# tphakala/birdnet-go

Hardware: AMD Instinct MI355X
Metric: 3s-48kHz clips/sec (whole node) + max-abs prob diff vs TFLite, BirdNET v2.4 (higher is better)
Workload: dtype f32; 1 GPU; BASELINE configs[1]: BirdNET v2.4 fp32, batch 256 x 3 s @ 48 kHz per GPU, mel front-end + CNN + head on device, raw logits out; batch_per_gpu=256, n_samples=144000, n_classes=6522, pipeline_depth=2, input_sets=4

## Files before the change

birdnet-go_amd/csrc/expdw.hip:

```cpp
#include "kernels.h"
#include "pw_common.h"

#include <algorithm>
#include <type_traits>
#include <cmath>
#include <cstdio>
#include <cstdlib>
#include <cstring>
#include <vector>

namespace bnhip {

struct ExpDwParams {
    const float* x; const float* we; const float* be; const float* wd; const float* bd;
    float* y; float* partial;
    int B, H, W, Cin, Cmid, Ho, Wo, pt, pl, act_e, act_d, tiles_h, tiles_w, cchunks, Kw, Cp;
    int Hin = 0, Win = 0, pts = 0, pls = 0;
    const uint16_t* wep = nullptr; int Kp = 0;
    int prec = 0;
    int xsh = 0, xsw = 1, ysh = 0, ysw = 1, tr = 0;
    int in_bf16 = 0, out_bf16 = 0;
    FDiv d_bpc{}, d_cch{}, d_tw{};
    int cpp = 0;
    FDiv d_part{};
// ... 48 lines not shown
            for (int j = 0; j < K; j++) w[j] = wds[(i * K + j) * 8 + c4];
#pragma unroll
            for (int a = 0; a < SH; a++) {
                const int fr = (ty * SH + a) * S + i;
                if (fr < vr0 || fr >= vr1 || oh0 + ty * SH + a >= p.Ho) continue;
                float4 xr[RW];
#pragma unroll
                for (int c = 0; c < RW; c++) xr[c] = *reinterpret_cast<const float4*>(e0 + ((fr - vr0) * TIW + c) * ED_ES);
#pragma unroll
                for (int j = 0; j < K; j++) {
#pragma unroll
                    for (int c = 0; c < SW; c++) {
                        const float4 xv = xr[c * S + j];
                        acc2[a][c].x = fmaf(xv.x, w[j].x, acc2[a][c].x); acc2[a][c].y = fmaf(xv.y, w[j].y, acc2[a][c].y);
                        acc2[a][c].z = fmaf(xv.z, w[j].z, acc2[a][c].z); acc2[a][c].w = fmaf(xv.w, w[j].w, acc2[a][c].w);
                    }
                }
            }
        }
    }
    pre_store();
    if (n < p.Cmid) {
        float* const yclip = p.y + (size_t)b * p.Ho * p.Wo * p.Cmid;
        const unsigned ylane = (unsigned)(((oh0 + ty * SH) * p.ysh + (ow0 + tx * SW) * p.ysw) * p.Cmid + n);
#pragma unroll
        for (int a = 0; a < SH; a++) {
            int oh = oh0 + ty * SH + a;
            if (oh >= p.Ho) continue;
            if (p.act_d == ACT_SWISH) {
#pragma unroll
                for (int c = 0; c < SW; c++) {
                    float4& v = acc2[a][c];
                    const f32x4 r = swish4((f32x4){v.x + bv.x, v.y + bv.y, v.z + bv.z, v.w + bv.w});
                    v = make_float4(r[0], r[1], r[2], r[3]);
                }
            } else {
                with_act(p.act_d, [&](auto f) {
#pragma unroll
                    for (int c = 0; c < SW; c++) {
                        float4& v = acc2[a][c];
                        v.x = f(v.x + bv.x); v.y = f(v.y + bv.y); v.z = f(v.z + bv.z); v.w = f(v.w + bv.w);
                    }
                });
            }
#pragma unroll
            for (int c = 0; c < SW; c++) {
                int ow = ow0 + tx * SW + c;
                if (ow >= p.Wo) continue;
                float4 v = acc2[a][c];
                const unsigned yo = ylane + (unsigned)((a * p.ysh + c * p.ysw) * p.Cmid);
                if (p.out_bf16) bf16x4_store(p.y, ((size_t)b * p.Ho * p.Wo * p.Cmid + yo) >> 2, v);
                else *reinterpret_cast<float4*>(yclip + yo) = v;
                sum.x += v.x; sum.y += v.y; sum.z += v.z; sum.w += v.w;
            }
        }
    }
    return sum;
}
__device__ __forceinline__ void ed_sums_lanes(float4 sum, float4* red, int wave, int lane, int c4) {
    static_assert(ed_perm_c4_rule(ED_PERM2) && ed_perm_c4_rule(ED_PERM4), "lane permutation: c4 bit 2 must be physical lane bit 3");
    auto xsum = [&](auto pat) {
        constexpr int P = decltype(pat)::value;
        sum.x += __builtin_bit_cast(float, __builtin_amdgcn_ds_swizzle(__builtin_bit_cast(int, sum.x), P));
        sum.y += __builtin_bit_cast(float, __builtin_amdgcn_ds_swizzle(__builtin_bit_cast(int, sum.y), P));
        sum.z += __builtin_bit_cast(float, __builtin_amdgcn_ds_swizzle(__builtin_bit_cast(int, sum.z), P));
        sum.w += __builtin_bit_cast(float, __builtin_amdgcn_ds_swizzle(__builtin_bit_cast(int, sum.w), P));
    };
    xsum(std::integral_constant<int, 0x101f>{});
    xsum(std::integral_constant<int, 0x401f>{});
    if ((lane & 0x14) == 0) red[(wave * 2 + (lane >> 5)) * 8 + c4] = sum;
}
template <int NW = 4>
__device__ __forceinline__ void ed_sums_out(const ExpDwParams& p, const float4* red, int tid, size_t tile_index, int n_base) {
    if (tid < 8 && n_base + 4 * tid < p.Cmid) {
        float4 t = red[tid];
#pragma unroll
        for (int w = 1; w < 2 * NW; w++) { float4 v = red[w * 8 + tid]; t.x += v.x; t.y += v.y; t.z += v.z; t.w += v.w; }
        unsigned l4 = 4u * (unsigned)tid;
        asm volatile("" : "+v"(l4));
        *reinterpret_cast<float4*>(p.partial + tile_index * p.Cmid + n_base + l4) = t;
    }
}

template <int K, int S, int TOH, int TOW, int TRH, bool H8 = false, bool BX = false, bool COPY = false>
__global__ __launch_bounds__(256, BX ? expdw_min_waves(K, S, TOW, TRH) : 1) void k_expand_dw(ExpDwParams p, unsigned nblk) {
    constexpr int TIH = (TOH - 1) * S + K, TIW = (TOW - 1) * S + K;
    static_assert(TRH <= TIH, "TRH is a cap on the footprint rows");
    constexpr int NPIX = TRH * TIW, NPIXP = (NPIX + 15) / 16 * 16;
    constexpr int JT = NPIXP / 16, JTW = (JT + 3) / 4;
    constexpr int SW = TOW / 8;
    __shared__ __attribute__((aligned(16))) float lds[NPIX * ED_ES + 256 + K * K * 32];
    float* E = lds;
    float4* red = reinterpret_cast<float4*>(lds + NPIX * ED_ES);
    float4* wds = reinterpret_cast<float4*>(lds + NPIX * ED_ES + 256);
    const int tid = threadIdx.x, lane = tid & 63, wave = __builtin_amdgcn_readfirstlane(tid >> 6);
    const int li = lane & 15, kq = lane >> 4;

    const unsigned L = xcd_remap(blockIdx.x, nblk);
    const int tiles = p.tiles_h * p.tiles_w;
    const int bpc = tiles * p.cchunks;
    const int b = (int)fdiv(L, p.d_bpc), rest = (int)L - b * bpc;
    const int tile = (int)fdiv((unsigned)rest, p.d_cch), cc = rest - tile * p.cchunks;
    const int trow = (int)fdiv((unsigned)tile, p.d_tw);
    const int oh0 = trow * TOH, ow0 = (tile - trow * p.tiles_w) * TOW;
    const int ih0 = oh0 * S - p.pt, iw0 = ow0 * S - p.pl;
    const int vr0 = max(ih0, 0) - ih0, vr1 = min(ih0 + TIH, p.H) - ih0;
    const int nvalid = (vr1 - vr0) * TIW;
    const int jtv = (nvalid + 15) >> 4;
    const int Cin = p.Cin, Kw = p.Kw;
    const int n_base = cc * 32;

    static_assert(SW * S == 2 || SW * S == 4, "lane permutation tables cover SW*S in {2, 4}");
    constexpr unsigned long long PERM = SW * S == 2 ? ED_PERM2 : ED_PERM4;
    const int pl = ed_perm(PERM, lane);
    const int c4 = pl & 7, tx = pl >> 3;
    float4 wdreg = make_float4(0.f, 0.f, 0.f, 0.f);
    if (tid < K * K * 8 && (!COPY || n_base + 4 * (tid & 7) < p.Cmid)) {
        const int tap = tid >> 3, tsrc = p.tr ? (tap % K) * K + tap / K : tap;
        wdreg = *reinterpret_cast<const float4*>(p.wd + (size_t)tsrc * p.Cp + n_base + 4 * (tid & 7));
    }
    const float4 zero4 = make_float4(0.f, 0.f, 0.f, 0.f);
    const float4 bq0 = COPY ? zero4 : *reinterpret_cast<const float4*>(p.be + n_base + 4 * kq);
    const float4 bq1 = COPY ? zero4 : *reinterpret_cast<const float4*>(p.be + n_base + 16 + 4 * kq);
    const float4 bv = (COPY && (!p.bd || n_base + 4 * c4 >= p.Cmid)) ? zero4 : *reinterpret_cast<const float4*>(p.bd + n_base + 4 * c4);

    if constexpr (COPY) {
        const float4* x4 = reinterpret_cast<const float4*>(p.x);
        const int C4 = p.Cmid >> 2, q4 = (n_base >> 2) + (tid & 7);
        const bool cin = q4 < C4;
        const size_t img = (size_t)b * p.H * p.W;
#pragma unroll 4
        for (int j = tid >> 3; j < nvalid; j += 32) {
            const int r = j / TIW, c = j - r * TIW;
            const int iw = iw0 + c, ih = ih0 + vr0 + r;
            float4 v = zero4;
            if (cin && iw >= 0 && iw < p.W) {
                const size_t quad = (img + (size_t)ih * p.xsh + (size_t)iw * p.xsw) * C4 + q4;
                v = p.in_bf16 ? bf16x4_load(p.x, quad) : x4[quad];
            }
            *reinterpret_cast<float4*>(&E[j * ED_ES + 4 * (tid & 7)]) = v;
        }
        if (tid < K * K * 8) wds[tid] = wdreg;
        __syncthreads();
    } else {

    int xoff[JTW];
    bool xin[JTW];
#pragma unroll
    for (int a = 0; a < JTW; a++) {
        int j = 16 * (wave + 4 * a) + li;
        int r = j / TIW, c = j - r * TIW;
        int iw = iw0 + c;
        xin[a] = j < nvalid && iw >= 0 && iw < p.W;
        int ihc = min(ih0 + vr0 + r, p.H - 1), iwc = min(max(iw, 0), p.W - 1);
        xoff[a] = (b * p.H * p.W + ihc * p.xsh + iwc * p.xsw) * Cin + (BX ? 8 : 4) * kq;
    }
    const float* wrow0 = p.we + (size_t)(n_base + li) * Kw + 4 * kq;
    const float* wrow1 = wrow0 + (size_t)16 * Kw;

    f32x4 acc[JTW][2];
#pragma unroll
    for (int a = 0; a < JTW; a++) { acc[a][0] = (f32x4){bq0.x, bq0.y, bq0.z, bq0.w}; acc[a][1] = (f32x4){bq1.x, bq1.y, bq1.z, bq1.w}; }

    auto fload = [&](int k0, f32x4& wf0, f32x4& wf1, f32x4 (&xf)[JTW]) {
        float4 t0 = *reinterpret_cast<const float4*>(wrow0 + k0), t1 = *reinterpret_cast<const float4*>(wrow1 + k0);
        wf0 = (f32x4){t0.x, t0.y, t0.z, t0.w}; wf1 = (f32x4){t1.x, t1.y, t1.z, t1.w};
        const int kx = (k0 + 4 * kq < Cin) ? k0 : -4 * kq;
#pragma unroll
        for (int a = 0; a < JTW; a++) {
            float4 t = *reinterpret_cast<const float4*>(p.x + (size_t)xoff[a] + kx);
            xf[a] = (f32x4){t.x, t.y, t.z, t.w};
        }
    };
    auto fmma = [&](const f32x4& wf0, const f32x4& wf1, const f32x4 (&xf)[JTW]) {
#pragma unroll
        for (int a = 0; a < JTW; a++) {
            if (wave + 4 * a < jtv) {
#pragma unroll
                for (int sidx = 0; sidx < 4; sidx++) {
                    acc[a][0] = __builtin_amdgcn_mfma_f32_16x16x4f32(wf0[sidx], xf[a][sidx], acc[a][0], 0, 0, 0);
                    acc[a][1] = __builtin_amdgcn_mfma_f32_16x16x4f32(wf1[sidx], xf[a][sidx], acc[a][1], 0, 0, 0);
                }
            }
        }
    };
    auto fload8 = [&](int k0, f32x2& wh0, f32x2& wh1, f32x2 (&xh)[JTW]) {
        const float2 t0 = *reinterpret_cast<const float2*>(wrow0 - 2 * kq + k0), t1 = *reinterpret_cast<const float2*>(wrow1 - 2 * kq + k0);
        wh0 = (f32x2){t0.x, t0.y}; wh1 = (f32x2){t1.x, t1.y};
        const int kx = (k0 + 2 * kq + 1 < Cin) ? k0 - 2 * kq : -4 * kq;
#pragma unroll
        for (int a = 0; a < JTW; a++) {
            const float2 t = *reinterpret_cast<const float2*>(p.x + (size_t)xoff[a] + kx);
            xh[a] = (f32x2){t.x, t.y};
        }
    };
    auto fmma8 = [&](const f32x2& wh0, const f32x2& wh1, const f32x2 (&xh)[JTW]) {
#pragma unroll
        for (int a = 0; a < JTW; a++) {
            if (wave + 4 * a < jtv) {
#pragma unroll
                for (int sidx = 0; sidx < 2; sidx++) {
                    acc[a][0] = __builtin_amdgcn_mfma_f32_16x16x4f32(wh0[sidx], xh[a][sidx], acc[a][0], 0, 0, 0);
                    acc[a][1] = __builtin_amdgcn_mfma_f32_16x16x4f32(wh1[sidx], xh[a][sidx], acc[a][1], 0, 0, 0);
                }
            }
        }
    };
    const int Kfull = Kw & ~15;
    if (BX) {
        const u32x4* wimg = reinterpret_cast<const u32x4*>(p.wep);
        const unsigned kp8 = (unsigned)p.Kp >> 3;
        const unsigned wr0 = (unsigned)(n_base + li) * 3u * kp8 + (unsigned)kq, wr1 = wr0 + 48u * kp8;
        for (int s32 = 0; s32 < (p.Kp >> 5); s32++) {
            const int kx = (32 * s32 + 8 * kq + 7 < Cin) ? 32 * s32 : -8 * kq;
            if (p.prec == 1) {
                const bf16x8 w0 = __builtin_bit_cast(bf16x8, wimg[wr0 + 4 * s32]), w1 = __builtin_bit_cast(bf16x8, wimg[wr1 + 4 * s32]);
#pragma unroll
                for (int a = 0; a < JTW; a++) {
                    if (wave + 4 * a < jtv) {
                        const float* xq = p.x + (size_t)xoff[a] + kx;
                        const float4 t0 = *reinterpret_cast<const float4*>(xq), t1 = *reinterpret_cast<const float4*>(xq + 4);
                        const bf16x8 xh = bx1_cvt8(t0, t1);
                        acc[a][0] = __builtin_amdgcn_mfma_f32_16x16x32_bf16(w0, xh, acc[a][0], 0, 0, 0);
                        acc[a][1] = __builtin_amdgcn_mfma_f32_16x16x32_bf16(w1, xh, acc[a][1], 0, 0, 0);
                    }
                }
                continue;
            }
            u32x4 wq[2][3];
#pragma unroll
            for (int pl3 = 0; pl3 < 3; pl3++) { wq[0][pl3] = wimg[wr0 + pl3 * kp8 + 4 * s32]; wq[1][pl3] = wimg[wr1 + pl3 * kp8 + 4 * s32]; }
#pragma unroll
            for (int a = 0; a < JTW; a++) {
                if (wave + 4 * a < jtv) {
                    const float* xq = p.x + (size_t)xoff[a] + kx;
                    const float4 t0 = *reinterpret_cast<const float4*>(xq), t1 = *reinterpret_cast<const float4*>(xq + 4);
                    bf16x8 xh, xm, xl;
                    bx3_split8(t0, t1, &xh, &xm, &xl);
#pragma unroll
                    for (int t = 0; t < 2; t++) {
                        acc[a][t] = bx3_mfma6(acc[a][t], __builtin_bit_cast(bf16x8, wq[t][0]), __builtin_bit_cast(bf16x8, wq[t][1]),
                                              __builtin_bit_cast(bf16x8, wq[t][2]), xh, xm, xl);
                    }
                }
            }
        }
    } else if (!H8) {
        for (int k0 = 0; k0 < Kw; k0 += 16) {
            f32x4 wf0, wf1, xf[JTW];
            fload(k0, wf0, wf1, xf);
            fmma(wf0, wf1, xf);
        }
    } else {
        for (int k0 = 0; k0 < Kfull; k0 += 16) {
            f32x4 wf0, wf1, xf[JTW];
            fload(k0, wf0, wf1, xf);
            fmma(wf0, wf1, xf);
        }
        f32x2 hA0, hA1, hx[JTW];
        fload8(Kfull, hA0, hA1, hx);
        fmma8(hA0, hA1, hx);
    }

    const bool border = iw0 < 0 || iw0 + TIW > p.W;
#pragma unroll
    for (int a = 0; a < JTW; a++) {
        if (wave + 4 * a < jtv) {
            if (p.act_e == ACT_SWISH) {
                acc[a][0] = swish4(acc[a][0]);
                acc[a][1] = swish4(acc[a][1]);
            } else {
                with_act(p.act_e, [&](auto f) {
                    f32x4& v0 = acc[a][0];
                    f32x4& v1 = acc[a][1];
                    v0[0] = f(v0[0]); v0[1] = f(v0[1]); v0[2] = f(v0[2]); v0[3] = f(v0[3]);
                    v1[0] = f(v1[0]); v1[1] = f(v1[1]); v1[2] = f(v1[2]); v1[3] = f(v1[3]);
                });
            }
            int j = 16 * (wave + 4 * a) + li;
            if (j < nvalid) {
                int e = j * ED_ES + 4 * kq;
                if (border) {
                    const f32x4 z = (f32x4){0.f, 0.f, 0.f, 0.f};
                    *reinterpret_cast<f32x4*>(&E[e]) = xin[a] ? acc[a][0] : z;
                    *reinterpret_cast<f32x4*>(&E[e + 16]) = xin[a] ? acc[a][1] : z;
                } else {
                    *reinterpret_cast<f32x4*>(&E[e]) = acc[a][0];
                    *reinterpret_cast<f32x4*>(&E[e + 16]) = acc[a][1];
                }
            }
        }
    }
    if (tid < K * K * 8) wds[tid] = wdreg;
    __syncthreads();
    }

    const float4 sum = ed_phase2<K, S, TOH, TOW, TRH, 4>(p, E, wds, b, oh0, ow0, vr0, vr1, wave, tx, c4, n_base, bv, [] {});
    if (p.partial) {
        ed_sums_lanes(sum, red, wave, lane, c4);
        __syncthreads();
        ed_sums_out(p, red, tid, (size_t)b * tiles + tile, n_base);
    }
}

template <int K, int S, int TOH, int TOW, int TRH, bool STEM, int KW, bool LOOP = !STEM, int NW = 4, int PH = 0, int NS = 1>
__global__ __launch_bounds__(64 * NW, expdw_sk_waves(K, S, TOH, TOW, TRH, PH == 1 ? 16 * NS : KW, !LOOP, NW)) void k_expand_dw_sk(ExpDwParams p, unsigned nblk) {
    static_assert(PH == 0 || PH == 1, "phase 1 on the f32 or on the bf16 pipe");
    constexpr bool B16 = PH == 1;
    static_assert(!B16 || (LOOP && !STEM), "bf16 phase 1: chunk-loop form");
    static_assert(NS == 1 || B16, "several resident slabs: bf16 operands only");
    constexpr int KP = 32 * NS;
    static_assert(PH != 1 || KW == 24 || KW == 32, "one-product form: layers of the bf16 engines");
    static_assert(NW == 4 || (NW == 8 && LOOP && TOH % 8 == 0), "eight-wave blocks: chunk-loop form, tile height a multiple of 8");
    static_assert(KW == 16 || KW == 24 || KW == 32, "one or two K slabs, or a slab and a half");
    static_assert(!STEM || KW == 24, "the stem's window is 3 rows x 4 columns x 2 channels");
    constexpr int TIH = (TOH - 1) * S + K, TIW = (TOW - 1) * S + K;
    static_assert(TRH <= TIH, "TRH is a cap on the footprint rows");
    constexpr int NPIX = TRH * TIW, NPIXP = (NPIX + 15) / 16 * 16;
    constexpr int JT = NPIXP / 16, JTW = (JT + NW - 1) / NW;
    constexpr int SW = TOW / 8;
    constexpr int NMMA = B16 ? 2 * NS : KW / 2;
    __shared__ __attribute__((aligned(16))) float lds[NPIX * ED_ES + 64 * NW + K * K * 32];
    float* E = lds;
    float4* red = reinterpret_cast<float4*>(lds + NPIX * ED_ES);
    float4* wds = reinterpret_cast<float4*>(lds + NPIX * ED_ES + 64 * NW);
    const int tid = threadIdx.x, lane = tid & 63, wave = __builtin_amdgcn_readfirstlane(tid >> 6);
    const int li = lane & 15, kq = lane >> 4;

    const unsigned L = xcd_remap(blockIdx.x, nblk);
    const int tiles = p.tiles_h * p.tiles_w;
    int b, tile, cc0 = 0;
    int cpp = p.cchunks;
    if constexpr (LOOP) {
        if (p.cpp > 0) {
            cpp = p.cpp;
            const int nparts = (p.cchunks + cpp - 1) / cpp;
            b = (int)fdiv(L, p.d_bpc);
            const int rest = (int)L - b * tiles * nparts;
            tile = (int)fdiv((unsigned)rest, p.d_part);
            cc0 = (rest - tile * nparts) * cpp;
        } else {
            b = (int)fdiv(L, p.d_bpc); tile = (int)L - b * tiles;
        }
    } else {
        b = (int)fdiv(L, p.d_bpc);
        const int rest = (int)L - b * tiles * p.cchunks;
        tile = (int)fdiv((unsigned)rest, p.d_cch); cc0 = rest - tile * p.cchunks;
    }
    const int trow = (int)fdiv((unsigned)tile, p.d_tw);
    const int oh0 = trow * TOH, ow0 = (tile - trow * p.tiles_w) * TOW;
    const int ih0 = oh0 * S - p.pt, iw0 = ow0 * S - p.pl;
    const int vr0 = max(ih0, 0) - ih0, vr1 = min(ih0 + TIH, p.H) - ih0;
    const int nvalid = (vr1 - vr0) * TIW;
    const int jtv = (nvalid + 15) >> 4;
    const int Cin = p.Cin;
    const int ncc = LOOP ? min(cpp, p.cchunks - cc0) : 1;
    const size_t tile_index = (size_t)b * tiles + tile;

    static_assert(SW * S == 2 || SW * S == 4, "lane permutation tables cover SW*S in {2, 4}");
    constexpr unsigned long long PERM = SW * S == 2 ? ED_PERM2 : ED_PERM4;
    const int pl = ed_perm(PERM, lane);
    const int c4 = pl & 7, tx = pl >> 3;

// ... 150 lines not shown
        };
        auto tile_out = [&](int a, auto masked, auto hi, auto&& act4) {
            constexpr bool HI = decltype(hi)::value;
            acc[a][0] = act4(acc[a][0]);
            if (HI) acc[a][1] = act4(acc[a][1]);
            if (16 * (wave + NW * a) + li < nvalid) {
                float* e = E + (16 * (wave + NW * a)) * ED_ES + e_lane;
                if constexpr (decltype(masked)::value) {
                    const f32x4 z = (f32x4){0.f, 0.f, 0.f, 0.f};
                    *reinterpret_cast<f32x4*>(e) = xin[a] ? acc[a][0] : z;
                    if (HI) *reinterpret_cast<f32x4*>(e + 16) = xin[a] ? acc[a][1] : z;
                } else {
                    *reinterpret_cast<f32x4*>(e) = acc[a][0];
                    if (HI) *reinterpret_cast<f32x4*>(e + 16) = acc[a][1];
                }
            }
        };
        auto phase1 = [&](auto masked, auto hi, auto&& act4) {
            if (wave < jtv) tile_mma(0, hi);
            if (LOOP && ci > 0) {
                __syncthreads();
                if (p.partial) ed_sums_out<NW>(p, red, tid, tile_index, n_base - 32);
            }
#pragma unroll
            for (int a = 1; a < JTW; a++) {
                if (wave + NW * a < jtv) {
                    tile_mma(a, hi);
                    tile_out(a - 1, masked, hi, act4);
#pragma unroll
                    for (int m = 0; m < (decltype(hi)::value ? NMMA : NMMA / 2); m++) {
                        __builtin_amdgcn_sched_group_barrier(0x008, 1, 0);
                        __builtin_amdgcn_sched_group_barrier(0x002, 2, 0);
                        __builtin_amdgcn_sched_group_barrier(0x400, 2, 0);
                    }
                } else if (wave + NW * (a - 1) < jtv) tile_out(a - 1, masked, hi, act4);
            }
            if (wave + NW * (JTW - 1) < jtv) tile_out(JTW - 1, masked, hi, act4);
        };
        auto phase1_act = [&](auto masked, auto hi) {
            if (LOOP || p.act_e == ACT_SWISH) phase1(masked, hi, [](f32x4 v) { return swish4(v); });
            else {
                const int act = p.act_e;
                phase1(masked, hi, [act](f32x4 v) {
                    return (f32x4){apply_act(v[0], act), apply_act(v[1], act), apply_act(v[2], act), apply_act(v[3], act)};
                });
            }
        };
        if (LOOP && n_base + 16 >= p.Cmid) {
            if (border) phase1_act(std::true_type{}, std::false_type{});
            else phase1_act(std::false_type{}, std::false_type{});
        } else {
            if (border) phase1_act(std::true_type{}, std::true_type{});
            else phase1_act(std::false_type{}, std::true_type{});
        }
        if (tid < K * K * 8) wds[tid] = q.wd;
        const float4 bv = q.bv;
        __syncthreads();
        if (LOOP && ci + 1 < ncc) fetch(cc + 1, q);

        const float4 sum = ed_phase2<K, S, TOH, TOW, TRH, NW>(p, E, wds, b, oh0, ow0, vr0, vr1, wave, tx, c4, n_base, bv, land);
        if (p.partial) ed_sums_lanes(sum, red, wave, lane, c4);
    }
    if (p.partial) {
        __syncthreads();
        ed_sums_out<NW>(p, red, tid, tile_index, (cc0 + ncc - 1) * 32);
    }
}

int expdw_kw(int Cin) { return (Cin & 1) ? (Cin + 15) / 16 * 16 : (Cin + 7) / 8 * 8; }
int expdw_skw(int Cin, int act_e, bool stem) {
    const int kw = expdw_kw(Cin);
    return !stem && act_e == ACT_SWISH && (kw == 16 || kw == 24 || kw == 32) ? kw : 0;
}
int expdw_cp(int Cmid) { return (Cmid + 31) / 32 * 32; }
struct ExpDwShape { int k, s, toh, tow, trh, nw = 4; };
static const ExpDwShape kExpDwShapes[] = {
    {3, 1, 8, 16, 10}, {3, 1, 4, 16, 6}, {3, 1, 8, 32, 6}, {3, 1, 8, 32, 10},
    {5, 1, 8, 16, 12}, {5, 1, 4, 16, 8}, {5, 1, 8, 32, 6}, {5, 1, 12, 16, 12},
    {3, 2, 4, 8, 9}, {3, 2, 8, 8, 12}, {3, 2, 8, 8, 17},
    {5, 2, 4, 8, 11}, {5, 2, 4, 16, 6}, {5, 2, 8, 8, 19},
    {3, 1, 8, 16, 10, 8}, {3, 1, 8, 32, 6, 8}, {3, 1, 8, 32, 10, 8}, {5, 1, 8, 16, 12, 8}, {5, 1, 8, 32, 6, 8},
    {3, 2, 8, 8, 12, 8}, {3, 2, 8, 8, 17, 8}, {5, 2, 8, 8, 19, 8},
};
static long expdw_cost(const ExpDwShape& sh, int H, int Ho, int Wo, int pt, bool* fits) {
    const int tih = (sh.toh - 1) * sh.s + sh.k, tiw = (sh.tow - 1) * sh.s + sh.k;
    const int th = (Ho + sh.toh - 1) / sh.toh, tw = (Wo + sh.tow - 1) / sh.tow;
    long rows = 0;
    *fits = true;
    for (int t = 0; t < th; t++) {
        int ih0 = t * sh.toh * sh.s - pt;
        int v = std::min(ih0 + tih, H) - std::max(ih0, 0);
        if (v > sh.trh) *fits = false;
        rows += std::max(v, 0);
    }
    return rows * tiw * tw;
}
static const int kNumExpDwShapes = (int)(sizeof(kExpDwShapes) / sizeof(kExpDwShapes[0]));
int expdw_num_shapes() { return 2 * kNumExpDwShapes; }
static ExpDwGeo expdw_oriented(int idx, const ExpDwGeo& g) {
    if (idx < kNumExpDwShapes) return g;
    ExpDwGeo t = g;
    t.H = g.W; t.W = g.H; t.Ho = g.Wo; t.Wo = g.Ho; t.pt = g.pl; t.pl = g.pt;
    return t;
}
bool expdw_shape_fits(int idx, const ExpDwGeo& g0, bool planning) {
    if (idx < 0 || idx >= 2 * kNumExpDwShapes) return false;
    if (idx >= kNumExpDwShapes && g0.stem) return false;
    if (!g0.stem && planning) {
        const char* oe = getenv("BNHIP_EXPDW_ORIENT");
        if (oe && ((oe[0] == 'n' && idx >= kNumExpDwShapes) || (oe[0] == 't' && idx < kNumExpDwShapes))) return false;
    }
    const ExpDwShape& sh = kExpDwShapes[idx % kNumExpDwShapes];
    if (sh.k != g0.k || sh.s != g0.s) return false;
    if (sh.nw == 8) {
        static const bool off = getenv("BNHIP_NO_EXPDW_NW8") != nullptr;
        if (off || g0.stem || !(g0.skw == 16 || g0.skw == 24 || g0.skw == 32)) return false;
    }
    const ExpDwGeo g = expdw_oriented(idx, g0);
    bool fits;
    (void)expdw_cost(sh, g.H, g.Ho, g.Wo, g.pt, &fits);
    return fits;
}
int expdw_shape_slabs(int idx, const ExpDwGeo& g0) {
    const ExpDwShape& sh = kExpDwShapes[idx % kNumExpDwShapes];
    const ExpDwGeo g = expdw_oriented(idx, g0);
    return ((g.Ho + sh.toh - 1) / sh.toh) * ((g.Wo + sh.tow - 1) / sh.tow);
}
int expdw_default_shape(const ExpDwGeo& g0) {
    int best = -1;
    long best_cost = 0;
    for (int i = 0; i < 2 * kNumExpDwShapes; i++) {
        if (!expdw_shape_fits(i, g0)) continue;
        const ExpDwGeo g = expdw_oriented(i, g0);
        const ExpDwShape& sh = kExpDwShapes[i % kNumExpDwShapes];
        bool fits;
        long c = expdw_cost(sh, g.H, g.Ho, g.Wo, g.pt, &fits);
        const long lds = (long)sh.trh * ((sh.tow - 1) * sh.s + sh.k) * ED_ES * 4;
        if (lds > 51 * 1024) c += c / 3;
        if (best < 0 || c < best_cost) { best = i; best_cost = c; }
    }
    return best;
}
int expdw_sum_slabs(const ExpDwGeo& g) {
    int idx = expdw_default_shape(g);
    return idx < 0 ? 0 : expdw_shape_slabs(idx, g);
}
int expdw_max_slabs(const ExpDwGeo& g) {
    int mx = 0;
    for (int i = 0; i < 2 * kNumExpDwShapes; i++)
        if (expdw_shape_fits(i, g)) mx = std::max(mx, expdw_shape_slabs(i, g));
    return mx;
}
bool expdw_bx_ok(int Cin) { return (Cin & 7) == 0 && Cin >= 16; }
int expdw_kp(int Cin) { return (Cin + 31) / 32 * 32; }
std::vector<uint16_t> expdw_bx_image(const float* We , int Cmid, int Cin) {
    const int Cp = expdw_cp(Cmid), Kp = expdw_kp(Cin);
    std::vector<uint16_t> img((size_t)Cp * 3 * Kp, 0);
    for (int n = 0; n < Cmid; n++)
        for (int k = 0; k < Cin; k++) {
            uint16_t piece[3];
            bx3_split_host(We[(size_t)n * Cin + k], piece);
            for (int pl = 0; pl < 3; pl++) img[((size_t)n * 3 + pl) * Kp + k] = piece[pl];
        }
    return img;
}
bool expdw_sk_pipe16(int Cin, int act_e, bool stem, int prec, bool have_image) {
    static const bool off = getenv("BNHIP_EXPDW_B16") && atoi(getenv("BNHIP_EXPDW_B16")) == 0;
    static const int max_ns = getenv("BNHIP_EXPDW_B16_NS") ? atoi(getenv("BNHIP_EXPDW_B16_NS")) : 5;
    if (off || !have_image || stem || act_e != ACT_SWISH || !expdw_bx_ok(Cin)) return false;
    const int kw = expdw_skw(Cin, act_e, stem), ns = expdw_kp(Cin) / 32;
    return prec == 1 && ((kw == 24 || kw == 32) || (kw == 0 && (ns == 2 || ns == 3 || ns == 5) && ns <= max_ns));
}
bool expdw_supported(int k, int s, int Cin, int Cmid, int act_e, int prec) {
    if (!((k == 3 || k == 5) && (s == 1 || s == 2) && (Cin & 3) == 0 && (Cmid & 3) == 0)) return false;
    if (Cin <= 128) return true;
    return prec == 1 && expdw_sk_pipe16(Cin, act_e, false, prec, true);
}
void launch_expand_dw(const float* x, const float* we, const float* be, const float* wd, const float* bd, float* y,
                      float* partial, int B, int H, int W, int Cin, int Cmid, int Ho, int Wo, int k, int s, int pt,
                      int pl, int act_e, int act_d, int shape, const StemGeom* stem, hipStream_t st, const uint16_t* wep, int prec, int out_bf16,
                      int in_bf16) {
    const bool pipe16 = expdw_sk_pipe16(Cin, act_e, stem != nullptr, prec, wep != nullptr);
    const ExpDwGeo g0{k, s, H, W, Ho, Wo, pt, pl, stem != nullptr, pipe16 ? 0 : expdw_skw(Cin, act_e, stem != nullptr)};
    if (!expdw_shape_fits(shape, g0, false)) shape = expdw_default_shape(g0);
    if (shape < 0) return;
    const ExpDwShape* sh = &kExpDwShapes[shape % kNumExpDwShapes];
    const bool tr = shape >= kNumExpDwShapes;
    const ExpDwGeo g = expdw_oriented(shape, g0);
    ExpDwParams p{x, we, be, wd, bd, y, partial, B, g.H, g.W, Cin, Cmid, g.Ho, g.Wo, g.pt, g.pl, act_e, act_d,
                  (g.Ho + sh->toh - 1) / sh->toh, (g.Wo + sh->tow - 1) / sh->tow, (Cmid + 31) / 32, expdw_kw(Cin), expdw_cp(Cmid)};
    p.xsh = tr ? 1 : W; p.xsw = tr ? W : 1; p.ysh = tr ? 1 : Wo; p.ysw = tr ? Wo : 1; p.tr = tr ? 1 : 0;
    p.out_bf16 = out_bf16;
    unsigned nblk = (unsigned)B * p.tiles_h * p.tiles_w * p.cchunks;
    p.d_bpc = make_fdiv((unsigned)(p.tiles_h * p.tiles_w * p.cchunks));
    p.d_cch = make_fdiv((unsigned)p.cchunks);
    p.d_tw = make_fdiv((unsigned)p.tiles_w);
    if (stem) p.Kw = 24;
    const bool sk = stem || pipe16 || (act_e == ACT_SWISH && (p.Kw == 16 || p.Kw == 24 || p.Kw == 32));
    const bool bx = wep != nullptr && !sk && expdw_bx_ok(Cin);
    if (bx) { p.wep = wep; p.Kp = expdw_kp(Cin); p.prec = prec; }
    const bool b16 = pipe16;
    if (pipe16) { p.wep = wep; p.Kp = expdw_kp(Cin); p.prec = prec; p.in_bf16 = in_bf16; }
    if (sk && !stem) {
        const int tiles = p.tiles_h * p.tiles_w;
        nblk = (unsigned)B * tiles;
        p.d_bpc = make_fdiv((unsigned)tiles);
        const int cus = device_cus();
        if (p.cchunks > 1 && (long)B * tiles < cus / 2) {
            const int want = (int)std::min<long>(p.cchunks, (cus + (long)B * tiles - 1) / ((long)B * tiles));
            const int cpp = (p.cchunks + want - 1) / want, nparts = (p.cchunks + cpp - 1) / cpp;
            if (nparts > 1) {
                p.cpp = cpp;
                p.d_part = make_fdiv((unsigned)nparts);
                nblk = (unsigned)B * tiles * nparts;
                p.d_bpc = make_fdiv((unsigned)(tiles * nparts));
            }
        }
    }
    if (stem) {
        p.Hin = stem->Hin; p.Win = stem->Win; p.pts = stem->pt; p.pls = stem->pl;
#define ED_STEM(TH_, TW_, TR_)                                                                                \
    if (sh->k == 3 && sh->s == 1 && sh->toh == TH_ && sh->tow == TW_ && sh->trh == TR_) {                     \
        hipLaunchKernelGGL((k_expand_dw_sk<3, 1, TH_, TW_, TR_, true, 24>), dim3(nblk), dim3(256), 0, st, p, nblk);  \
        return;                                                                                               \
    }
        ED_STEM(8, 16, 10) ED_STEM(4, 16, 6) ED_STEM(8, 32, 6) ED_STEM(8, 32, 10)
#undef ED_STEM
        return;
    }
#define ED_CASE8(K_, S_, TH_, TW_, TR_)                                                                       \
    if (sh->nw == 8 && sh->k == K_ && sh->s == S_ && sh->toh == TH_ && sh->tow == TW_ && sh->trh == TR_) {    \
        if (p.Kw == 16) hipLaunchKernelGGL((k_expand_dw_sk<K_, S_, TH_, TW_, TR_, false, 16, true, 8>), dim3(nblk), dim3(512), 0, st, p, nblk); \
        else if (p.Kw == 24) hipLaunchKernelGGL((k_expand_dw_sk<K_, S_, TH_, TW_, TR_, false, 24, true, 8>), dim3(nblk), dim3(512), 0, st, p, nblk); \
        else hipLaunchKernelGGL((k_expand_dw_sk<K_, S_, TH_, TW_, TR_, false, 32, true, 8>), dim3(nblk), dim3(512), 0, st, p, nblk); \
        return;                                                                                               \
    }
    if (sh->nw == 8) {
        if (!sk || stem) return;
        ED_CASE8(3, 1, 8, 16, 10) ED_CASE8(3, 1, 8, 32, 6) ED_CASE8(3, 1, 8, 32, 10) ED_CASE8(5, 1, 8, 16, 12) ED_CASE8(5, 1, 8, 32, 6)
        ED_CASE8(3, 2, 8, 8, 12) ED_CASE8(3, 2, 8, 8, 17) ED_CASE8(5, 2, 8, 8, 19)
        return;
    }
#undef ED_CASE8
#define ED_CASE(K_, S_, TH_, TW_, TR_)                                                                        \
    if (sh->k == K_ && sh->s == S_ && sh->toh == TH_ && sh->tow == TW_ && sh->trh == TR_) {                   \
        if (bx) hipLaunchKernelGGL((k_expand_dw<K_, S_, TH_, TW_, TR_, false, true>), dim3(nblk), dim3(256), 0, st, p, nblk); \
        else if (b16 && p.Kp == 64) hipLaunchKernelGGL((k_expand_dw_sk<K_, S_, TH_, TW_, TR_, false, 32, true, 4, 1, 2>), dim3(nblk), dim3(256), 0, st, p, nblk); \
        else if (b16 && p.Kp == 96) hipLaunchKernelGGL((k_expand_dw_sk<K_, S_, TH_, TW_, TR_, false, 32, true, 4, 1, 3>), dim3(nblk), dim3(256), 0, st, p, nblk); \
        else if (b16 && p.Kp == 160) hipLaunchKernelGGL((k_expand_dw_sk<K_, S_, TH_, TW_, TR_, false, 32, true, 4, 1, 5>), dim3(nblk), dim3(256), 0, st, p, nblk); \
        else if (b16 && p.Kw == 24) hipLaunchKernelGGL((k_expand_dw_sk<K_, S_, TH_, TW_, TR_, false, 24, true, 4, 1>), dim3(nblk), dim3(256), 0, st, p, nblk); \
        else if (b16) hipLaunchKernelGGL((k_expand_dw_sk<K_, S_, TH_, TW_, TR_, false, 32, true, 4, 1>), dim3(nblk), dim3(256), 0, st, p, nblk); \
        else if (sk && p.Kw == 16) hipLaunchKernelGGL((k_expand_dw_sk<K_, S_, TH_, TW_, TR_, false, 16>), dim3(nblk), dim3(256), 0, st, p, nblk); \
        else if (sk && p.Kw == 24) hipLaunchKernelGGL((k_expand_dw_sk<K_, S_, TH_, TW_, TR_, false, 24>), dim3(nblk), dim3(256), 0, st, p, nblk); \
        else if (sk && p.Kw == 32) hipLaunchKernelGGL((k_expand_dw_sk<K_, S_, TH_, TW_, TR_, false, 32>), dim3(nblk), dim3(256), 0, st, p, nblk); \
        else if (p.Kw & 8) hipLaunchKernelGGL((k_expand_dw<K_, S_, TH_, TW_, TR_, true>), dim3(nblk), dim3(256), 0, st, p, nblk); \
        else hipLaunchKernelGGL((k_expand_dw<K_, S_, TH_, TW_, TR_>), dim3(nblk), dim3(256), 0, st, p, nblk);  \
        return;                                                                                               \
    }
    ED_CASE(3, 1, 8, 16, 10) ED_CASE(3, 1, 4, 16, 6) ED_CASE(3, 1, 8, 32, 6) ED_CASE(3, 1, 8, 32, 10)
    ED_CASE(5, 1, 8, 16, 12) ED_CASE(5, 1, 4, 16, 8) ED_CASE(5, 1, 8, 32, 6) ED_CASE(5, 1, 12, 16, 12)
    ED_CASE(3, 2, 4, 8, 9) ED_CASE(3, 2, 8, 8, 12) ED_CASE(3, 2, 8, 8, 17)
    ED_CASE(5, 2, 4, 8, 11) ED_CASE(5, 2, 4, 16, 6) ED_CASE(5, 2, 8, 8, 19)
#undef ED_CASE
}

bool dwconv_lds_supported(const DwParams& p) {
    return (p.C & 3) == 0 && p.kh == p.kw && p.sh == p.sw && (p.kh == 3 || p.kh == 5) && (p.sh == 1 || p.sh == 2);
}
void launch_dwconv_lds(const DwParams& q, float* partial, int shape, hipStream_t st) {
    const ExpDwGeo g0{q.kh, q.sh, q.H, q.W, q.Ho, q.Wo, q.pt, q.pl, false};
    if (!expdw_shape_fits(shape, g0, false)) shape = expdw_default_shape(g0);
    if (shape < 0) return;
    const ExpDwShape* sh = &kExpDwShapes[shape % kNumExpDwShapes];
    const bool tr = shape >= kNumExpDwShapes;
    const ExpDwGeo g = expdw_oriented(shape, g0);
    ExpDwParams p{q.in, nullptr, nullptr, q.w, q.bias, q.out, partial, q.B, g.H, g.W, q.C, q.C, g.Ho, g.Wo, g.pt, g.pl, ACT_NONE, q.act,
                  (g.Ho + sh->toh - 1) / sh->toh, (g.Wo + sh->tow - 1) / sh->tow, (q.C + 31) / 32, 0, q.C};
    p.xsh = tr ? 1 : q.W; p.xsw = tr ? q.W : 1; p.ysh = tr ? 1 : q.Wo; p.ysw = tr ? q.Wo : 1; p.tr = tr ? 1 : 0;
    p.in_bf16 = q.in_bf16; p.out_bf16 = q.out_bf16;
    unsigned nblk = (unsigned)q.B * p.tiles_h * p.tiles_w * p.cchunks;
    p.d_bpc = make_fdiv((unsigned)(p.tiles_h * p.tiles_w * p.cchunks));
    p.d_cch = make_fdiv((unsigned)p.cchunks);
    p.d_tw = make_fdiv((unsigned)p.tiles_w);
#define DL_CASE(K_, S_, TH_, TW_, TR_)                                                                        \
    if (sh->k == K_ && sh->s == S_ && sh->toh == TH_ && sh->tow == TW_ && sh->trh == TR_) {                   \
        hipLaunchKernelGGL((k_expand_dw<K_, S_, TH_, TW_, TR_, false, false, true>), dim3(nblk), dim3(256), 0, st, p, nblk); \
        return;                                                                                               \
    }
    DL_CASE(3, 1, 8, 16, 10) DL_CASE(3, 1, 4, 16, 6) DL_CASE(3, 1, 8, 32, 6) DL_CASE(3, 1, 8, 32, 10)
    DL_CASE(5, 1, 8, 16, 12) DL_CASE(5, 1, 4, 16, 8) DL_CASE(5, 1, 8, 32, 6) DL_CASE(5, 1, 12, 16, 12)
    DL_CASE(3, 2, 4, 8, 9) DL_CASE(3, 2, 8, 8, 12) DL_CASE(3, 2, 8, 8, 17)
    DL_CASE(5, 2, 4, 8, 11) DL_CASE(5, 2, 4, 16, 6) DL_CASE(5, 2, 8, 8, 19)
#undef DL_CASE
}


}
```

birdnet-go_amd/csrc/kernels.h:

```cpp
#pragma once
#include <atomic>
#include <hip/hip_runtime.h>

#include <vector>
#include <cstdint>

namespace bnhip {

inline int device_cus() {
    static std::atomic<int> cus[64];
    int dev = 0;
    if (hipGetDevice(&dev) != hipSuccess) { (void)hipGetLastError(); return 256; }
    if (dev < 0 || dev >= 64) return 256;
    int c = cus[dev].load(std::memory_order_relaxed);
    if (c > 0) return c;
    hipDeviceProp_t pr{};
    if (hipGetDeviceProperties(&pr, dev) != hipSuccess || pr.multiProcessorCount <= 0) { (void)hipGetLastError(); return 256; }
    cus[dev].store(pr.multiProcessorCount, std::memory_order_relaxed);
    return pr.multiProcessorCount;
}

struct PwGrid { int nblk_n; unsigned nblk; };
inline PwGrid pw_grid(int M, int N, int nt, int wm) {
    const int nblk_n = (N + nt * 16 - 1) / (nt * 16);
// ... 80 lines not shown
    float lfloor = 0.f, lscale = 1.f;
    int time_major = 0;
};
bool mel_banded_supported(int n_mels, int nbp0, int nbp1);
void launch_mel_banded(const MelBandParams& p, int nch, int n_clips, hipStream_t s);
int frontend_kc(int Lfft, int hop, int NTP);

struct ConvParams {
    const float* in; const float* w ; const float* bias; float* out;
    int B, H, W, Cin, Ho, Wo, Cout, kh, kw, sh, sw, pt, pl, act;
    int out_bf16 = 0;
};
void launch_conv_direct(const ConvParams& p, hipStream_t s);
bool conv_direct_bf16_ok(const ConvParams& p);
bool conv_igemm_supported(int Cin, int Cout, int kh, int kw);
void launch_conv_igemm(const float* in, const float* w_ohwi, const float* bias, float* out, int B, int H, int W, int Cin, int Ho, int Wo,
                       int Cout, int kh, int kw, int sh, int sw, int dh, int dw, int pt, int pl, int act, int nt ,
                       int wm , hipStream_t s);
bool stem_mfma_supported(const ConvParams& p);
void launch_stem_mfma(const ConvParams& p, const float* wm, const float* bias_p, hipStream_t s);

struct PwParams {
    const float* A; const float* W; const float* bias; const float* ascale; const float* res; float* out;
    int M, N, K, HW, act;
    int nt = 0;
    int wm = 0;
    int prec = 0;
    int a_bf16 = 0;
    int out_bf16 = 0;
    int res_bf16 = 0;
    int sw = 0;
};
enum { PW_SW_B16_OFF = 1, PW_SW_B16_FORCE = 2, PW_SW_B16S_OFF = 4, PW_SW_B16S_FORCE = 8, PW_SW_WS_OFF = 16, PW_SW_WS_FORCE = 32, PW_SW_LAT_OFF = 64,
       PW_SW_TAIL_OFF = 128, PW_SW_TAIL_FORCE = 256 };
int pw_switches_from_env();
void launch_pw_gemm(const PwParams& p, hipStream_t s);
bool pw_pipe_ok(int nt, int wm, int K);
int pw_default_nt(int M, int N);
bool pw_bx3_ok(int K);
bool pw_bx3p_ok(int nt, int wm , int K);
int pw_bx3_npad(int N);
std::vector<uint16_t> pw_bx3_image(const float* W, int N, int K);
void launch_pw_bx3(const PwParams& p, const uint16_t* Wimg, hipStream_t s);
bool pw_b16_ok(int prec, int K, int sw);
struct PwTail {
    int kind = 0;
    int H = 0, W = 0;
    int k = 0, pt = 0, pl = 0, act = 0;
    const float* w = nullptr; const float* bias = nullptr;
    float* out = nullptr;
    float* partial = nullptr;
    int PY = 0, tiles_w = 0, tiles = 0, tchunks = 0;
};
int pw_tail_rows(int wm);
bool pw_tail_ok(const PwParams& p, const PwTail& t, int nt, int wm);
bool pw_tail_fills(const PwParams& p, int nt, int wm);
void launch_pw_tail(const PwParams& p, const PwTail& t, const uint16_t* Wimg, int nt, int wm, hipStream_t s);
bool pw_b16s_ok(const PwParams& p);
void launch_pw_b16s(const PwParams& p, const uint16_t* Wimg, int Npad, hipStream_t s);
void launch_pw_b16(const PwParams& p, const uint16_t* Wimg, int nt, int wm , int Npad, int nblk_n, unsigned nblk, hipStream_t s);
bool pw_lat_ok(const PwParams& p);
void launch_pw_lat(const PwParams& p, const uint16_t* Wimg, int Npad, hipStream_t s);
bool pw_ws_ok(const PwParams& p);
bool pw_ws_fills(const PwParams& p);
void launch_pw_ws(const PwParams& p, const uint16_t* Wimg, int Npad, hipStream_t s);

struct DwParams {
    const float* in; const float* w ; const float* bias; float* out;
    int B, H, W, C, Ho, Wo, kh, kw, sh, sw, pt, pl, act;
    int in_bf16 = 0, out_bf16 = 0;
};
int dwconv_sum_slabs(const DwParams& p);
bool dwconv_tile_geometry(const DwParams& p, int* PY, int* tiles_w, int* tiles, int* tchunks);
void launch_dwconv(const DwParams& p, float* partial, hipStream_t s);

bool expdw_supported(int k, int s, int Cin, int Cmid, int act_e = 0, int prec = 0);
struct ExpDwGeo { int k, s, H, W, Ho, Wo, pt, pl; bool stem = false; int skw = 0; };
int expdw_skw(int Cin, int act_e, bool stem);
bool expdw_sk_pipe16(int Cin, int act_e, bool stem, int prec, bool have_image);
int expdw_sum_slabs(const ExpDwGeo& g);
int expdw_num_shapes();
bool expdw_shape_fits(int idx, const ExpDwGeo& g, bool planning = true);
int expdw_shape_slabs(int idx, const ExpDwGeo& g);
int expdw_default_shape(const ExpDwGeo& g);
int expdw_max_slabs(const ExpDwGeo& g);
struct StemGeom { int Hin, Win, pt, pl; };
int expdw_kw(int Cin);
int expdw_cp(int Cmid);
void launch_expand_dw(const float* x, const float* we, const float* be, const float* wd, const float* bd, float* y,
                      float* partial, int B, int H, int W, int Cin, int Cmid, int Ho, int Wo, int k, int s, int pt,
                      int pl, int act_e, int act_d, int shape ,
                      const StemGeom* stem ,
                      hipStream_t st, const uint16_t* wep = nullptr ,
                      int prec = 0 ,
                      int out_bf16 = 0 ,
                      int in_bf16 = 0 );
bool dwconv_lds_supported(const DwParams& p);
void launch_dwconv_lds(const DwParams& p, float* partial, int shape, hipStream_t st);
bool expdw_bx_ok(int Cin);
int expdw_kp(int Cin);
std::vector<uint16_t> expdw_bx_image(const float* We , int Cmid, int Cin);

int mean_splits(int HW);
int mean_partial_py(int C);
void launch_mean_partial(const float* in, float* partial, int B, int HW, int C, int S, hipStream_t s);
void launch_mean_finish(const float* partial, float* out, int B, int HW, int C, int S, hipStream_t s);

struct SeParams {
    const float* partial; int S; int HW;
    const float* w1; const float* b1;
    const float* w2; const float* b2;
    float* scale;
    int B, C, Cr, act1, act2;
    int threads = 0;
};
void launch_se(const SeParams& p, hipStream_t s);

void launch_unary(const float* in, float* out, size_t n, int act, hipStream_t s);
void launch_binary(const float* a, const float* b, float* out, size_t n, int op , int mode,
                   int HW, int C, int act, hipStream_t s);

enum UnaryOp : int { U_ABS = 200, U_SQRT, U_RSQRT, U_LOG, U_EXP, U_NEG, U_SQUARE, U_TANH, U_LEAKY_RELU, U_ELU, U_SIN, U_COS,
                     U_FLOOR, U_CEIL, U_ROUND, U_RELU_N1_TO_1, U_LOGISTIC, U_RELU, U_RELU6, U_HARD_SWISH, U_GELU, U_GELU_TANH };
enum BinaryOp : int { B_ADD = 0, B_MUL = 1, B_SUB = 2, B_DIV = 3, B_POW = 4, B_MAX = 5, B_MIN = 6, B_SQDIFF = 7 };
enum ReduceOp : int { R_SUM = 0, R_MEAN = 1, R_MAX = 2, R_MIN = 3, R_PROD = 4 };
void launch_unary_op(const float* in, float* out, size_t n, int op, float alpha, hipStream_t s);
struct BcastParams {
    const float* a; const float* b; float* out;
    int d[4]; long sa[4], sb[4]; long bsa, bsb;
    int op, act;
};
void launch_binary_bcast(const BcastParams& p, int n_clips, hipStream_t s);
struct CopyParams {
    const float* in; float* out;
    int d[4]; long si[4], so[4]; long offi, offo, bsi, bso;
};
void launch_copy_view(const CopyParams& p, int n_clips, hipStream_t s);
void launch_fill(float* out, size_t n, float v, hipStream_t s);
struct PoolParams { const float* in; float* out; int B, H, W, C, Ho, Wo, kh, kw, sh, sw, pt, pl, mode , act; };
void launch_pool2d(const PoolParams& p, hipStream_t s);
void launch_softmax_rows(const float* in, float* out, size_t rows, int n, float beta, hipStream_t s);
struct ReduceParams { const float* in; float* out; int d[4]; int mask ; int op; };
void launch_reduce(const ReduceParams& p, int n_clips, hipStream_t s);
struct GenConvParams {
    const float* in; const float* w; const float* bias; float* out;
    int B, H, W, Cin, Ho, Wo, Cout, kh, kw, sh, sw, dh, dw, pt, pl, act, depthwise, mult;
};
void launch_conv_generic(const GenConvParams& p, hipStream_t s);

void launch_activation(const float* logits, float* conf, int n_clips, int n_classes, int activation, double sens,
                       hipStream_t s);
void launch_topk(const float* conf, int n_clips, int n_classes, int k, float* out_conf, int32_t* out_idx,
                 hipStream_t s);

std::vector<double> us_twiddle_table(int fft_size);
void launch_us_frame_power(const void* samples , int pcm16, int n_clips, int n, int fft_size,
                           int hop, int frames, int split_bin, const double* d_tw, double* powers , hipStream_t s);
void launch_us_cv(const double* powers, int n_clips, int frames, double* cv, hipStream_t s);

}
```

Before: 76680 clips/s.

## Add full-width expand+depthwise variant that skips padded-column expand work

Adds a templated full-width mode (VW>0) to the fused expand+depthwise kernel, used when the whole image width equals 32 and fits in one tile. The expand GEMM then runs only over the valid width columns instead of the padded footprint width, and the padding columns in LDS are zero-filled with one float4 store per thread. This drops per-element border checks and clamping. The cost model also accounts for the narrower footprint when choosing shapes. It adds template instantiations and an environment switch to disable it, and is correct only for the exact geometry that expdw_fullw_geo checks.

```diff
diff --git a/birdnet-go_amd/csrc/expdw.hip b/birdnet-go_amd/csrc/expdw.hip
--- a/birdnet-go_amd/csrc/expdw.hip
+++ b/birdnet-go_amd/csrc/expdw.hip
@@ -154,12 +154,17 @@
     }
 }
 
-template <int K, int S, int TOH, int TOW, int TRH, bool H8 = false, bool BX = false, bool COPY = false>
+constexpr int expdw_fullw_vw(int K, int S, int TOW) { return TOW * S == 32 && (TOW - 1) * S + K >= 32 ? 32 : 0; }
+template <int K, int S, int TOH, int TOW, int TRH, bool H8 = false, bool BX = false, bool COPY = false, int VW = 0>
 __global__ __launch_bounds__(256, BX ? expdw_min_waves(K, S, TOW, TRH) : 1) void k_expand_dw(ExpDwParams p, unsigned nblk) {
     constexpr int TIH = (TOH - 1) * S + K, TIW = (TOW - 1) * S + K;
     static_assert(TRH <= TIH, "TRH is a cap on the footprint rows");
-    constexpr int NPIX = TRH * TIW, NPIXP = (NPIX + 15) / 16 * 16;
-    constexpr int JT = NPIXP / 16, JTW = (JT + 3) / 4;
+    constexpr bool FULLW = VW > 0;
+    static_assert(!FULLW || (!COPY && VW % 16 == 0 && VW <= TIW && VW == expdw_fullw_vw(K, S, TOW)), "full-width form: see expdw_fullw_vw");
+    static_assert(!FULLW || (TIW - VW) * TRH * 8 <= 256, "full-width form: the padding columns are one float4 store of some threads");
+    constexpr int NPIX = TRH * TIW;
+    constexpr int GW = FULLW ? VW : TIW;
+    constexpr int JT = (TRH * GW + 15) / 16, JTW = (JT + 3) / 4;
     constexpr int SW = TOW / 8;
     __shared__ __attribute__((aligned(16))) float lds[NPIX * ED_ES + 256 + K * K * 32];
     float* E = lds;
@@ -177,7 +182,7 @@
     const int oh0 = trow * TOH, ow0 = (tile - trow * p.tiles_w) * TOW;
     const int ih0 = oh0 * S - p.pt, iw0 = ow0 * S - p.pl;
     const int vr0 = max(ih0, 0) - ih0, vr1 = min(ih0 + TIH, p.H) - ih0;
-    const int nvalid = (vr1 - vr0) * TIW;
+    const int nvalid = (vr1 - vr0) * GW;
     const int jtv = (nvalid + 15) >> 4;
     const int Cin = p.Cin, Kw = p.Kw;
     const int n_base = cc * 32;
@@ -217,15 +222,24 @@
     } else {
 
     int xoff[JTW];
-    bool xin[JTW];
+    bool xin[FULLW ? 1 : JTW];
 #pragma unroll
     for (int a = 0; a < JTW; a++) {
         int j = 16 * (wave + 4 * a) + li;
-        int r = j / TIW, c = j - r * TIW;
-        int iw = iw0 + c;
-        xin[a] = j < nvalid && iw >= 0 && iw < p.W;
-        int ihc = min(ih0 + vr0 + r, p.H - 1), iwc = min(max(iw, 0), p.W - 1);
+        int r = j / GW, c = j - r * GW;
+        int ihc = min(ih0 + vr0 + r, p.H - 1), iwc = c;
+        if constexpr (!FULLW) {
+            int iw = iw0 + c;
+            xin[a] = j < nvalid && iw >= 0 && iw < p.W;
+            iwc = min(max(iw, 0), p.W - 1);
+        }
         xoff[a] = (b * p.H * p.W + ihc * p.xsh + iwc * p.xsw) * Cin + (BX ? 8 : 4) * kq;
+    }
+    if constexpr (FULLW) {
+        constexpr int PC = TIW - VW;
+        const int pr = (tid >> 3) / PC, pc = (tid >> 3) - pr * PC;
+        if (PC > 0 && pr < vr1 - vr0)
+            *reinterpret_cast<float4*>(&E[(pr * TIW + (pc < p.pl ? pc : pc + VW)) * ED_ES + 4 * (tid & 7)]) = zero4;
     }
     const float* wrow0 = p.we + (size_t)(n_base + li) * Kw + 4 * kq;
     const float* wrow1 = wrow0 + (size_t)16 * Kw;
@@ -334,7 +348,7 @@
         fmma8(hA0, hA1, hx);
     }
 
-    const bool border = iw0 < 0 || iw0 + TIW > p.W;
+    const bool border = !FULLW && (iw0 < 0 || iw0 + TIW > p.W);
 #pragma unroll
     for (int a = 0; a < JTW; a++) {
         if (wave + 4 * a < jtv) {
@@ -350,7 +364,11 @@
                 });
             }
             int j = 16 * (wave + 4 * a) + li;
-            if (j < nvalid) {
+            if constexpr (FULLW) {
+                int e = ((j / VW) * TIW + j % VW + p.pl) * ED_ES + 4 * kq;
+                *reinterpret_cast<f32x4*>(&E[e]) = acc[a][0];
+                *reinterpret_cast<f32x4*>(&E[e + 16]) = acc[a][1];
+            } else if (j < nvalid) {
                 int e = j * ED_ES + 4 * kq;
                 if (border) {
                     const f32x4 z = (f32x4){0.f, 0.f, 0.f, 0.f};
@@ -667,8 +685,12 @@
     {3, 1, 8, 16, 10, 8}, {3, 1, 8, 32, 6, 8}, {3, 1, 8, 32, 10, 8}, {5, 1, 8, 16, 12, 8}, {5, 1, 8, 32, 6, 8},
     {3, 2, 8, 8, 12, 8}, {3, 2, 8, 8, 17, 8}, {5, 2, 8, 8, 19, 8},
 };
-static long expdw_cost(const ExpDwShape& sh, int H, int Ho, int Wo, int pt, bool* fits) {
-    const int tih = (sh.toh - 1) * sh.s + sh.k, tiw = (sh.tow - 1) * sh.s + sh.k;
+static bool expdw_fullw_geo(const ExpDwShape& sh, int W, int Wo, int pl) {
+    const int vw = expdw_fullw_vw(sh.k, sh.s, sh.tow), tiw = (sh.tow - 1) * sh.s + sh.k;
+    return sh.nw == 4 && vw > 0 && W == vw && Wo <= sh.tow && pl >= 0 && pl + vw <= tiw;
+}
+static long expdw_cost(const ExpDwShape& sh, int H, int W, int Ho, int Wo, int pt, int pl, bool* fits) {
+    const int tih = (sh.toh - 1) * sh.s + sh.k, tiw = expdw_fullw_geo(sh, W, Wo, pl) ? W : (sh.tow - 1) * sh.s + sh.k;
     const int th = (Ho + sh.toh - 1) / sh.toh, tw = (Wo + sh.tow - 1) / sh.tow;
     long rows = 0;
     *fits = true;
@@ -703,8 +725,15 @@
     }
     const ExpDwGeo g = expdw_oriented(idx, g0);
     bool fits;
-    (void)expdw_cost(sh, g.H, g.Ho, g.Wo, g.pt, &fits);
+    (void)expdw_cost(sh, g.H, g.W, g.Ho, g.Wo, g.pt, g.pl, &fits);
     return fits;
+}
+bool expdw_fullwidth(int idx, const ExpDwGeo& g0) {
+    static const bool off = getenv("BNHIP_EXPDW_FULLW") && atoi(getenv("BNHIP_EXPDW_FULLW")) == 0;
+    if (off || idx < 0 || idx >= 2 * kNumExpDwShapes || g0.stem || g0.skw != 0) return false;
+    const ExpDwShape& sh = kExpDwShapes[idx % kNumExpDwShapes];
+    const ExpDwGeo g = expdw_oriented(idx, g0);
+    return sh.k == g0.k && sh.s == g0.s && expdw_fullw_geo(sh, g.W, g.Wo, g.pl);
 }
 int expdw_shape_slabs(int idx, const ExpDwGeo& g0) {
     const ExpDwShape& sh = kExpDwShapes[idx % kNumExpDwShapes];
@@ -719,7 +748,7 @@
         const ExpDwGeo g = expdw_oriented(i, g0);
         const ExpDwShape& sh = kExpDwShapes[i % kNumExpDwShapes];
         bool fits;
-        long c = expdw_cost(sh, g.H, g.Ho, g.Wo, g.pt, &fits);
+        long c = expdw_cost(sh, g.H, g.W, g.Ho, g.Wo, g.pt, g.pl, &fits);
         const long lds = (long)sh.trh * ((sh.tow - 1) * sh.s + sh.k) * ED_ES * 4;
         if (lds > 51 * 1024) c += c / 3;
         if (best < 0 || c < best_cost) { best = i; best_cost = c; }
@@ -760,6 +789,17 @@
     if (!((k == 3 || k == 5) && (s == 1 || s == 2) && (Cin & 3) == 0 && (Cmid & 3) == 0)) return false;
     if (Cin <= 128) return true;
     return prec == 1 && expdw_sk_pipe16(Cin, act_e, false, prec, true);
+}
+template <int K, int S, int TH, int TW, int TR, bool H8, bool BX>
+static void ed_launch(const ExpDwParams& p, unsigned nblk, hipStream_t st, bool fullw) {
+    constexpr int VW = expdw_fullw_vw(K, S, TW);
+    if constexpr (VW > 0) {
+        if (fullw) {
+            hipLaunchKernelGGL((k_expand_dw<K, S, TH, TW, TR, H8, BX, false, VW>), dim3(nblk), dim3(256), 0, st, p, nblk);
+            return;
+        }
+    }
+    hipLaunchKernelGGL((k_expand_dw<K, S, TH, TW, TR, H8, BX>), dim3(nblk), dim3(256), 0, st, p, nblk);
 }
 void launch_expand_dw(const float* x, const float* we, const float* be, const float* wd, const float* bd, float* y,
                       float* partial, int B, int H, int W, int Cin, int Cmid, int Ho, int Wo, int k, int s, int pt,
@@ -785,6 +825,7 @@
     const bool bx = wep != nullptr && !sk && expdw_bx_ok(Cin);
     if (bx) { p.wep = wep; p.Kp = expdw_kp(Cin); p.prec = prec; }
     const bool b16 = pipe16;
+    const bool fullw = !sk && expdw_fullwidth(shape, g0);
     if (pipe16) { p.wep = wep; p.Kp = expdw_kp(Cin); p.prec = prec; p.in_bf16 = in_bf16; }
     if (sk && !stem) {
         const int tiles = p.tiles_h * p.tiles_w;
@@ -829,7 +870,7 @@
 #undef ED_CASE8
 #define ED_CASE(K_, S_, TH_, TW_, TR_)                                                                        \
     if (sh->k == K_ && sh->s == S_ && sh->toh == TH_ && sh->tow == TW_ && sh->trh == TR_) {                   \
-        if (bx) hipLaunchKernelGGL((k_expand_dw<K_, S_, TH_, TW_, TR_, false, true>), dim3(nblk), dim3(256), 0, st, p, nblk); \
+        if (bx) ed_launch<K_, S_, TH_, TW_, TR_, false, true>(p, nblk, st, fullw);                                \
         else if (b16 && p.Kp == 64) hipLaunchKernelGGL((k_expand_dw_sk<K_, S_, TH_, TW_, TR_, false, 32, true, 4, 1, 2>), dim3(nblk), dim3(256), 0, st, p, nblk); \
         else if (b16 && p.Kp == 96) hipLaunchKernelGGL((k_expand_dw_sk<K_, S_, TH_, TW_, TR_, false, 32, true, 4, 1, 3>), dim3(nblk), dim3(256), 0, st, p, nblk); \
         else if (b16 && p.Kp == 160) hipLaunchKernelGGL((k_expand_dw_sk<K_, S_, TH_, TW_, TR_, false, 32, true, 4, 1, 5>), dim3(nblk), dim3(256), 0, st, p, nblk); \
@@ -838,8 +879,8 @@
         else if (sk && p.Kw == 16) hipLaunchKernelGGL((k_expand_dw_sk<K_, S_, TH_, TW_, TR_, false, 16>), dim3(nblk), dim3(256), 0, st, p, nblk); \
         else if (sk && p.Kw == 24) hipLaunchKernelGGL((k_expand_dw_sk<K_, S_, TH_, TW_, TR_, false, 24>), dim3(nblk), dim3(256), 0, st, p, nblk); \
         else if (sk && p.Kw == 32) hipLaunchKernelGGL((k_expand_dw_sk<K_, S_, TH_, TW_, TR_, false, 32>), dim3(nblk), dim3(256), 0, st, p, nblk); \
-        else if (p.Kw & 8) hipLaunchKernelGGL((k_expand_dw<K_, S_, TH_, TW_, TR_, true>), dim3(nblk), dim3(256), 0, st, p, nblk); \
-        else hipLaunchKernelGGL((k_expand_dw<K_, S_, TH_, TW_, TR_>), dim3(nblk), dim3(256), 0, st, p, nblk);  \
+        else if (p.Kw & 8) ed_launch<K_, S_, TH_, TW_, TR_, true, false>(p, nblk, st, fullw);                     \
+        else ed_launch<K_, S_, TH_, TW_, TR_, false, false>(p, nblk, st, fullw);                                  \
         return;                                                                                               \
     }
     ED_CASE(3, 1, 8, 16, 10) ED_CASE(3, 1, 4, 16, 6) ED_CASE(3, 1, 8, 32, 6) ED_CASE(3, 1, 8, 32, 10)
diff --git a/birdnet-go_amd/csrc/kernels.h b/birdnet-go_amd/csrc/kernels.h
--- a/birdnet-go_amd/csrc/kernels.h
+++ b/birdnet-go_amd/csrc/kernels.h
@@ -186,6 +186,7 @@
 int expdw_num_shapes();
 bool expdw_shape_fits(int idx, const ExpDwGeo& g, bool planning = true);
 int expdw_shape_slabs(int idx, const ExpDwGeo& g);
+bool expdw_fullwidth(int idx, const ExpDwGeo& g);
 int expdw_default_shape(const ExpDwGeo& g);
 int expdw_max_slabs(const ExpDwGeo& g);
 struct StemGeom { int Hin, Win, pt, pl; };
```

After: 78170 clips/s, median of 6. +1.9%, better.
